# marcelm/cutadapt

Measured on NVIDIA H100. Metric: reads/sec (150bp SE, 1 adapter, e=0.1), higher is better.
Workload: dtype u8

## Files before the change

cutadapt_b200/csrc/cg_core.cuh:

```cuda
#pragma once
#include "cg_types.h"

#define CGK_KIND_ALIGNER 0
#define CGK_KIND_PREFIX 1
#define CGK_KIND_SUFFIX 2
#define CGK_REMOVE_BEFORE 0
#define CGK_REMOVE_AFTER 1
#define CGK_REMOVE_AUTO 2
#define CGK_GROUP_SINGLE 0
#define CGK_GROUP_LINKED 1
#define CGK_GROUP_INDEXED 2

CG_HD int cg_ctz(uint32_t x)
{
#if defined(__CUDA_ARCH__)
    return __ffs((int)x) - 1;
#else
    return __builtin_ctz(x);
#endif
}
CG_HD uint32_t cg_funnel_r(uint32_t lo, uint32_t hi, uint32_t shift_bits)
{
#if defined(__CUDA_ARCH__)
    return __funnelshift_r(lo, hi, shift_bits);
// ... 1697 lines not shown
    locate_regs<MR>(A, ncnt, maxcost, peq, rv, R, R.n, has_task, !split, st);
    if (!has_task) return true;
    if (split && !st.stopped) return false;
    hit_from_state(A, n, st, hit);
    return true;
}

template <int MR>
CG_HD void split_end_pass(const SetView &S, const uint8_t *tail, int n, bool has_task, LocState &st, CgHit &hit)
{
    const CgAdapter &A = S.ad[0];
    const int lo_end = cg_max(0, n - 1 - A.m - A.k);
    ReadView rv;
    rv.n = n; rv.rev = A.reverse;
    rv.p = A.reverse ? tail : tail - lo_end;
    const int32_t *ncnt = (const int32_t *)(S.pool + A.ncount_off);
    const int32_t *maxcost = (const int32_t *)(S.pool + A.maxcost_off);
    const uint32_t *peq = (const uint32_t *)(S.pool + A.peq_off);
    RunList R;
    R.n = 1; R.lo0 = lo_end; R.hi0 = n; R.lo1 = R.hi1 = R.lo2 = R.hi2 = 0;
    locate_regs<MR>(A, ncnt, maxcost, peq, rv, R, 1, has_task, true, st, false);
    if (has_task) hit_from_state(A, n, st, hit);
}

CG_HD void process_read_simple(const SetView &S, const uint8_t *seq, const uint8_t *qual, int n,
                               int quality_trim, int cutoff_front, int cutoff_back, int qbase,
                               PackedCol &colp, cg_match_rec *out, int32_t *qtrim_out, int use_regs = 0)
{
    int s = 0, e = n;
    if (quality_trim) pre_trim_core(seq, qual, n, quality_trim, cutoff_front, cutoff_back, qbase, &s, &e);
    if (qtrim_out) { qtrim_out[0] = s; qtrim_out[1] = e; }
    CgHit hit; hit.adapter = -1; hit.remove = 0;
    hit.astart = hit.astop = hit.rstart = hit.rstop = hit.score = hit.errors = 0;
    if (use_regs == 3 && S.ad[0].m <= 32) {
        int gs3;
        const ScanOut sc3 = simple_scan(S, seq + s, e - s, &gs3);
        if (sc3.pass) {
            LocState st;
            const CgAdapter &A = S.ad[0];
            const int nn = e - s, lo_end = cg_max(0, nn - 1 - A.m - A.k);
            const uint8_t *tail = A.reverse ? seq + s : seq + s + lo_end;
            if (A.m <= 16) {
                if (!split_main_pass<16>(S, seq + s, nn, sc3.hits, gs3, sc3.rs0, sc3.rs1, true, hit, st))
                    split_end_pass<16>(S, tail, nn, true, st, hit);
            } else {
                if (!split_main_pass<32>(S, seq + s, nn, sc3.hits, gs3, sc3.rs0, sc3.rs1, true, hit, st))
                    split_end_pass<32>(S, tail, nn, true, st, hit);
            }
        }
        store_hit(out, hit, 0, e - s);
        return;
    }
    if (use_regs == 2 && S.ad[0].m <= 32) {
        RunList R;
        if (simple_scan_runs(S, seq + s, e - s, R)) {
            if (!simple_locate_runs(S, seq + s, e - s, R, true, hit)) hit.adapter = -1;
        }
        store_hit(out, hit, 0, e - s);
        return;
    }
    int gs;
    const ScanOut sc = simple_scan(S, seq + s, e - s, &gs);
    if (sc.pass) {
        const bool found = (use_regs && S.ad[0].m <= 32)
                               ? simple_locate_regs(S, seq + s, e - s, sc.hits, gs, sc.rs0, sc.rs1, true, hit)
                               : simple_locate(S, seq + s, e - s, sc.hits, gs, colp, hit);
        if (!found) hit.adapter = -1;
    }
    store_hit(out, hit, 0, e - s);
}




struct RunPlan {
    int n_runs;
    int lo0, hi0, lo1, hi1, lo2, hi2, lo3, hi3;
    int end_idx;
    int exact;
    int s0;
    int banded;
};

CG_HD int run_band_d(const CgAdapter &A, int n, int lo, int hi, bool hit_derived, bool is_end_run)
{
    const bool can = A.m <= 64 && !(A.flags & 1) && (A.flags & 2) && (A.flags & 8) && A.indel_cost == 1;
    if (!can || !hit_derived || is_end_run || hi >= n) return -1;
    const int d = hi - A.m - A.k - lo;
    return d >= 0 ? d : -1;
}

template <bool REV>
CG_HD void plan_hit_runs_dir(const CgScanWord *words, int n_words, const uint8_t *pool, const CgAdapter &A,
                             const uint8_t *first, int n, uint32_t hits, int gs, uint32_t rs0, uint32_t rs1,
                             bool want_exact, RunList &R, int &exact, int &s0_out)
{
    const int m = A.m, k = A.k;
    R.n = 0;
    R.lo0 = R.hi0 = R.lo1 = R.hi1 = R.lo2 = R.hi2 = 0;
    exact = 0; s0_out = 0;
    if (A.flags & 1) runs_add(R, 0, cg_min(n, m + k), n);
    if (!hits) return;
    int n_loc = 0;
    for (int w = 0; w < n_words; ++w) n_loc += (words[w].type == CG_SCAN_WHOLE && words[w].loc_found) ? 1 : 0;
    bool ex_ok = want_exact;
    int ex_s0 = -1;
    for (int w = 0; w < n_words; ++w) {
        const CgScanWord &W = words[w];
        if (W.type != CG_SCAN_WHOLE || !W.loc_found) continue;
        CG_TABPTR(mask, (const uint32_t *)(pool + W.mask_off));
        CG_CHARPTR(ltab, pool + W.loc_off);
        const uint32_t init = W.init, locf = W.loc_found;
        const bool stash = n_loc == 1;
        uint32_t todo = hits, Rr = 0;
        int cur_p = -1, nh = 0, stretch = 0;
        int wlo = 0x3fffffff, whi = -1;
        int s0 = 0x3fffffff;
        uint32_t fm = 0;
        while (todo) {
            const int g = cg_ctz(todo);
            todo &= todo - 1;
            const int p_first = g << gs;
            const long long p_end_ll = ((long long)(g + 1)) << gs;
            const int p_end = p_end_ll > n ? n : (int)p_end_ll;
            if (cur_p != p_first) {
                if (cur_p >= 0) ++stretch;
                if (whi >= 0) { runs_add(R, wlo, whi, n); wlo = 0x3fffffff; whi = -1; }
                if (stash && nh < 2) {
                    Rr = nh == 0 ? rs0 : rs1;
                } else {
                    Rr = 0;
                    const int q0 = cg_max(0, p_first - 31);
                    CG_CHARPTR(q, first + (REV ? -q0 : q0));
                    for (int i = q0; i < p_first; ++i) {
                        Rr = ((Rr << 1) | init) & CG_TAB32(mask, CG_CHAR(q));
                        q = REV ? q - 1 : q + 1;
                    }
                }
            }
            ++nh;
            uint32_t q0 = 0, q1 = 0, q2 = 0, q3 = 0, qpa = 0, qpb = 0;
            int qn = 0;
            auto handle = [&](int p, uint32_t f) {
                while (f) {
                    const int b = cg_ctz(f);
                    f &= f - 1;
                    const int bmin = (int)CG_CHAR(ltab + 2 * b), bmax = (int)CG_CHAR(ltab + 2 * b + 1);
                    wlo = cg_min(wlo, p + 1 - bmax - k);
                    whi = cg_max(whi, p + 1 - bmin + m + k);
                    if (stretch == 0) {
                        const int s = p + 1 - bmin;
                        if (s < s0) { s0 = s; fm = 1u << b; }
                        else if (s == s0) fm |= 1u << b;
                    }
                }
            };
            auto flush = [&]() {
                for (int e = qn - 1; e >= 0; --e) {
                    const uint32_t f = e == 3 ? q3 : (e == 2 ? q2 : (e == 1 ? q1 : q0));
                    const uint32_t pw = e >= 2 ? qpb : qpa;
                    handle((int)((e & 1) ? (pw >> 16) : (pw & 0xffffu)), f);
                }
                qn = 0;
            };
            auto push = [&](int p, uint32_t f) {
                if (qn == 4) flush();
                q3 = q2; q2 = q1; q1 = q0; q0 = f;
                qpb = (qpb << 16) | (qpa >> 16);
                qpa = (qpa << 16) | (uint32_t)p;
                ++qn;
            };
            CG_CHARPTR(q, first + (REV ? -p_first : p_first));
            for (int p = p_first; p < p_end; ++p) {
                Rr = ((Rr << 1) | init) & CG_TAB32(mask, CG_CHAR(q));
                q = REV ? q - 1 : q + 1;
                const uint32_t f = Rr & locf;
                if (f) push(p, f);
            }
            flush();
            cur_p = p_end;
        }
        if (whi >= 0) runs_add(R, wlo, whi, n);
        if (fm == locf && s0 >= 0 && s0 + m <= n && (ex_s0 < 0 || ex_s0 == s0)) ex_s0 = s0;
        else ex_ok = false;
    }
    if (ex_ok && ex_s0 >= 0) { exact = 1; s0_out = ex_s0; }
}

template <class T>
CG_HD void plan_runs_myers_t(const CgAdapter &A, const uint32_t *peq, const int32_t *ncnt,
                             const int32_t *maxcost, const uint8_t *p, int n, RunList &R, bool &need_end)
{
    const int m = A.m, k = A.k;
    const bool sir = (A.flags & 1) != 0, eir = (A.flags & 4) != 0;
    const T mmask = m >= (int)(8 * sizeof(T)) ? (T) ~(T)0 : (T)(((T)1 << m) - 1);
    const T top = (T)1 << (m - 1);
    T Pv = sir ? (T)0 : mmask, Mv = 0;
    int score = sir ? 0 : m;
    CG_CHARPTR(cp, A.reverse ? p + (n - 1) : p);
    CG_TABPTR(peq_t, peq);
    const int cstride = A.reverse ? -1 : 1;
    int wlo = 0, whi = -1;
    for (int j = 1; j <= n; ++j) {
        const int ch = (int)(CG_CHAR(cp + cstride * (j - 1)) & 127u);
        T Eq = (T)CG_TAB32(peq_t, ch);
        if (sizeof(T) > 4) Eq |= (T)((unsigned long long)CG_TAB32(peq_t, 128 + ch) << 32);
        const T Xv = Eq | Mv;
        const T Xh = (T)((((Eq & Pv) + Pv) ^ Pv) | Eq);
        T Ph = (T)(Mv | ~(Xh | Pv));
        T Mh = Pv & Xh;
        score += (Ph & top) ? 1 : 0;
        score -= (Mh & top) ? 1 : 0;
        Ph = (T)(Ph << 1); Mh = (T)(Mh << 1);
        Pv = (T)(Mh | ~(Xv | Ph));
        Mv = Ph & Xv;
        if (score <= k) {
            const int lo = cg_max(0, j - m - k);
            if (whi < 0) wlo = lo;
            else if (lo > whi) { runs_add(R, wlo, whi, n); wlo = lo; }
            whi = j;
        }
    }
    if (whi >= 0) runs_add(R, wlo, whi, n);
    need_end = false;
    if (eir) {
        if (sir) need_end = true;
        else {
            int c = 0;
            for (int i = 1; i <= m; ++i) {
                c += (int)((Pv >> (i - 1)) & 1) - (int)((Mv >> (i - 1)) & 1);
                int eff = i;
                if (A.wildcard_ref) eff = (i < m) ? i - ncnt[i] : A.effective_length;
                if (i >= A.min_overlap && c <= maxcost[eff]) { need_end = true; break; }
            }
        }
    }
}

template <class T>
CG_HD int end_overlap_myers_t(const CgAdapter &A, const uint32_t *peq, const int32_t *ncnt,
                              const int32_t *maxcost, const uint8_t *p, int n, int lo_end)
{
    const int m = A.m;
    const T mmask = m >= (int)(8 * sizeof(T)) ? (T) ~(T)0 : (T)(((T)1 << m) - 1);
    T Pv = mmask, Mv = 0;
    CG_CHARPTR(cp, A.reverse ? p + (n - 1) : p);
    CG_TABPTR(peq_t, peq);
    const int cstride = A.reverse ? -1 : 1;
    for (int j = lo_end + 1; j <= n; ++j) {
        const int ch = (int)(CG_CHAR(cp + cstride * (j - 1)) & 127u);
        T Eq = (T)CG_TAB32(peq_t, ch);
        if (sizeof(T) > 4) Eq |= (T)((unsigned long long)CG_TAB32(peq_t, 128 + ch) << 32);
        const T Xv = Eq | Mv;
        const T Xh = (T)((((Eq & Pv) + Pv) ^ Pv) | Eq);
        T Ph = (T)(Mv | ~(Xh | Pv));
        T Mh = Pv & Xh;
        Ph = (T)(Ph << 1); Mh = (T)(Mh << 1);
        Pv = (T)(Mh | ~(Xv | Ph));
        Mv = Ph & Xv;
    }
    int c = 0, best = 0;
    bool inexact = false;
    for (int i = 1; i <= m; ++i) {
        c += (int)((Pv >> (i - 1)) & 1) - (int)((Mv >> (i - 1)) & 1);
        int eff = i;
        if (A.wildcard_ref) eff = (i < m) ? i - ncnt[i] : A.effective_length;
        if (i >= A.min_overlap && c <= maxcost[eff]) {
            if (c == 0) best = i; else inexact = true;
        }
    }
    return inexact ? -1 : best;
}

template <class T>
CG_HD bool run_has_candidate_t(const CgAdapter &A, const uint32_t *peq, const uint8_t *p, int n, int lo, int hi)
{
    const int m = A.m, k = A.k;
    const T mmask = m >= (int)(8 * sizeof(T)) ? (T) ~(T)0 : (T)(((T)1 << m) - 1);
    const T top = (T)1 << (m - 1);
    T Pv = mmask, Mv = 0;
    int score = m;
    CG_CHARPTR(cp, A.reverse ? p + (n - 1) : p);
    CG_TABPTR(peq_t, peq);
    const int cstride = A.reverse ? -1 : 1;
    bool any = false;
    for (int j = lo + 1; j <= hi; ++j) {
        const int ch = (int)(CG_CHAR(cp + cstride * (j - 1)) & 127u);
        T Eq = (T)CG_TAB32(peq_t, ch);
        if (sizeof(T) > 4) Eq |= (T)((unsigned long long)CG_TAB32(peq_t, 128 + ch) << 32);
        const T Xv = Eq | Mv;
        const T Xh = (T)((((Eq & Pv) + Pv) ^ Pv) | Eq);
        T Ph = (T)(Mv | ~(Xh | Pv));
        T Mh = Pv & Xh;
        score += (Ph & top) ? 1 : 0;
        score -= (Mh & top) ? 1 : 0;
        Ph = (T)(Ph << 1); Mh = (T)(Mh << 1);
        Pv = (T)(Mh | ~(Xv | Ph));
        Mv = Ph & Xv;
        any = any || score <= k;
    }
    return any;
}

CG_HD void plan_finish(const SetView &S, const uint8_t *p, int n, const RunList &R0, RunPlan &P, bool skip_end = false)
{
    const CgAdapter &A = S.ad[0];
    const int32_t *ncnt = (const int32_t *)(S.pool + A.ncount_off);
    const int32_t *maxcost = (const int32_t *)(S.pool + A.maxcost_off);
    const uint32_t *peq = (const uint32_t *)(S.pool + A.peq_off);
    const bool eir = (A.flags & 4) != 0;
    const int lo_end = cg_max(0, n - 1 - A.m - A.k);
    const bool can_filter = A.m <= 64 && !(A.flags & 1) && (A.flags & 2) && (A.flags & 8) && A.indel_cost == 1;
    RunList R;
    R.n = 0; R.lo0 = R.hi0 = R.lo1 = R.hi1 = R.lo2 = R.hi2 = 0;
    bool covered = false;
    for (int r = 0; r < R0.n; ++r) {
        const int lo = r == 0 ? R0.lo0 : (r == 1 ? R0.lo1 : R0.lo2);
        const int hi = r == 0 ? R0.hi0 : (r == 1 ? R0.hi1 : R0.hi2);
        const bool is_final = eir && r == R0.n - 1 && lo <= lo_end && hi == n;
        bool keep = true;
        if (can_filter && !is_final)
            keep = A.m <= 32 ? run_has_candidate_t<uint32_t>(A, peq, p, n, lo, hi)
                             : run_has_candidate_t<unsigned long long>(A, peq, p, n, lo, hi);
        if (!keep) continue;
        if (R.n == 0) { R.lo0 = lo; R.hi0 = hi; }
        else if (R.n == 1) { R.lo1 = lo; R.hi1 = hi; }
        else { R.lo2 = lo; R.hi2 = hi; }
        ++R.n;
        covered = is_final;
    }
    P.n_runs = R.n; P.lo0 = R.lo0; P.hi0 = R.hi0; P.lo1 = R.lo1; P.hi1 = R.hi1; P.lo2 = R.lo2; P.hi2 = R.hi2;
    if (!eir || covered || skip_end) return;
    if (can_filter) {
        const int r = A.m <= 32 ? end_overlap_myers_t<uint32_t>(A, peq, ncnt, maxcost, p, n, lo_end)
                                : end_overlap_myers_t<unsigned long long>(A, peq, ncnt, maxcost, p, n, lo_end);
        if (r == 0) return;
        if (r > 0 && R.n == 0) { P.exact = 2; P.s0 = r; return; }
    }
    P.end_idx = R.n;
    if (R.n == 0) { P.lo0 = lo_end; P.hi0 = n; }
    else if (R.n == 1) { P.lo1 = lo_end; P.hi1 = n; }
    else if (R.n == 2) { P.lo2 = lo_end; P.hi2 = n; }
    else { P.lo3 = lo_end; P.hi3 = n; }
    P.n_runs = R.n + 1;
}

CG_HD void plan_runs(const SetView &S, const uint8_t *p, int n, uint32_t hits, int gs, uint32_t rs0,
                     uint32_t rs1, RunPlan &P)
{
    const CgAdapter &A = S.ad[0];
    P.n_runs = 0; P.lo0 = P.hi0 = P.lo1 = P.hi1 = P.lo2 = P.hi2 = P.lo3 = P.hi3 = 0;
    P.end_idx = -1; P.exact = 0; P.s0 = 0; P.banded = 0;
    if (S.h->myers && (A.flags & 2) && (A.flags & 8) && n > 0) {
        const int32_t *ncnt = (const int32_t *)(S.pool + A.ncount_off);
        const int32_t *maxcost = (const int32_t *)(S.pool + A.maxcost_off);
        const uint32_t *peq = (const uint32_t *)(S.pool + A.peq_off);
        RunList R;
        R.n = 0; R.lo0 = R.hi0 = R.lo1 = R.hi1 = R.lo2 = R.hi2 = 0;
        bool need_end;
        if (A.m <= 32) plan_runs_myers_t<uint32_t>(A, peq, ncnt, maxcost, p, n, R, need_end);
        else plan_runs_myers_t<unsigned long long>(A, peq, ncnt, maxcost, p, n, R, need_end);
        P.n_runs = R.n; P.lo0 = R.lo0; P.hi0 = R.hi0; P.lo1 = R.lo1; P.hi1 = R.hi1; P.lo2 = R.lo2; P.hi2 = R.hi2;
        if (need_end) {
            const int lo_end = cg_max(0, n - 1 - A.m - A.k);
            bool covered = false;
            if (R.n > 0) {
                const int lo_last = R.n == 1 ? R.lo0 : (R.n == 2 ? R.lo1 : R.lo2);
                const int hi_last = R.n == 1 ? R.hi0 : (R.n == 2 ? R.hi1 : R.hi2);
                covered = lo_last <= lo_end && hi_last == n;
            }
            if (!covered) {
                P.end_idx = R.n;
                if (R.n == 0) { P.lo0 = lo_end; P.hi0 = n; }
                else if (R.n == 1) { P.lo1 = lo_end; P.hi1 = n; }
                else if (R.n == 2) { P.lo2 = lo_end; P.hi2 = n; }
                else { P.lo3 = lo_end; P.hi3 = n; }
                P.n_runs = R.n + 1;
            }
        }
        return;
    }
    if (!simple_windowed(S, n)) {
        int max_n = n, min_n = 0;
        if (!(A.flags & 2)) max_n = cg_min(n, A.m + A.k);
        if (!(A.flags & 8)) min_n = cg_max(0, n - A.m - A.k);
        P.n_runs = 1; P.lo0 = min_n; P.hi0 = max_n;
        return;
    }
    RunList R;
    const bool want_exact = S.h->exact_ok != 0;
    if (A.reverse) plan_hit_runs_dir<true>(S.scan, S.h->scan_count, S.pool, A, p + (n - 1), n, hits, gs, rs0, rs1, want_exact, R, P.exact, P.s0);
    else plan_hit_runs_dir<false>(S.scan, S.h->scan_count, S.pool, A, p, n, hits, gs, rs0, rs1, want_exact, R, P.exact, P.s0);
    if (P.exact) return;
    plan_finish(S, p, n, R, P);
}

CG_HD bool window_is_plain(const uint8_t *p, int n)
{
    if (n <= 0) return true;
    const uint32_t mis = (uint32_t)((uintptr_t)p & 3u);
    const int total = n + (int)mis;
    const int n_words = (total + 3) >> 2;
#if defined(__CUDA_ARCH__)
    const uint32_t base = (uint32_t)__cvta_generic_to_shared(p - mis);
#define CG_PLAIN_WORD(i) cg_lds_u32(base + 4u * (uint32_t)(i))
#else
    const uint8_t *base = p - mis;
#define CG_PLAIN_WORD(i) ((uint32_t)base[4 * (i)] | ((uint32_t)base[4 * (i) + 1] << 8) | ((uint32_t)base[4 * (i) + 2] << 16) | \
                          ((uint32_t)base[4 * (i) + 3] << 24))
#endif
    uint32_t hi_or = 0, lo_or = 0, six_and = 0xFFFFFFFFu;
    auto take = [&](uint32_t w) {
        const uint32_t s1 = w >> 1, s2 = w >> 2, s4 = w >> 4;
        hi_or |= w & 0x88888888u;
        six_and &= w;
        lo_or |= ((s2 & ~s1) ^ s4) | ~(w ^ s4);
    };
    uint32_t keep0 = 0xFFFFFFFFu << (8 * mis);
    const uint32_t keep_last = (total & 3) ? 0xFFFFFFFFu >> (8 * (4 - (total & 3))) : 0xFFFFFFFFu;
    if (n_words == 1) keep0 &= keep_last;
    take((CG_PLAIN_WORD(0) & keep0) | (0x41414141u & ~keep0));
#pragma unroll 4
    for (int i = 1; i < n_words - 1; ++i) take(CG_PLAIN_WORD(i));
    if (n_words > 1) take((CG_PLAIN_WORD(n_words - 1) & keep_last) | (0x41414141u & ~keep_last));
#undef CG_PLAIN_WORD
    return hi_or == 0 && (six_and & 0x40404040u) == 0x40404040u && (lo_or & 0x01010101u) == 0;
}

CG_HD void plan_runs_planes(const SetView &S, const uint8_t *p, int n, const uint32_t *M, int W, int end_hit,
                            int no_end, int off0, RunPlan &P)
{
    const CgAdapter &A = S.ad[0];
    P.n_runs = 0; P.lo0 = P.hi0 = P.lo1 = P.hi1 = P.lo2 = P.hi2 = P.lo3 = P.hi3 = 0;
    P.end_idx = -1; P.exact = 0; P.s0 = 0; P.banded = 1;
    RunList R;
    R.n = 0; R.lo0 = R.hi0 = R.lo1 = R.hi1 = R.lo2 = R.hi2 = 0;
    if (A.flags & 1) runs_add(R, 0, cg_min(n, A.m + A.k), n);
#pragma unroll
    for (int b = 0; b < 8; ++b) {
        uint32_t x = b < W ? M[b] : 0u;
        while (x) {
            const int e = 32 * b + cg_ctz(x);
            x &= x - 1;
            const int s = e - (A.m - 1) - off0;
            runs_add(R, s - A.k, s + A.m + A.k, n);
        }
    }
    if (end_hit) runs_add(R, cg_max(0, n - 1 - A.m - A.k), n, n);
    plan_finish(S, p, n, R, P, no_end != 0 && !end_hit);
}

CG_HD void hit_end_overlap(const CgAdapter &A, int n, int len, CgHit &hit)
{
    LocState st = loc_state_init(A.m, n);
    st.have = 1; st.b_origin = n - len; st.b_cost = 0; st.b_score = len; st.b_ref_stop = len; st.b_q_stop = n;
    hit_from_state(A, n, st, hit);
}

CG_HD void hit_exact(const CgAdapter &A, int n, int s0, CgHit &hit)
{
    hit.adapter = 0;
    if (A.reverse) { hit.astart = 0; hit.astop = A.m; hit.rstart = n - (s0 + A.m); hit.rstop = n - s0; }
    else { hit.astart = 0; hit.astop = A.m; hit.rstart = s0; hit.rstop = s0 + A.m; }
    hit.score = A.m; hit.errors = 0;
    hit.remove = A.remove == CGK_REMOVE_AUTO ? (hit.rstart == 0 ? CGK_REMOVE_BEFORE : CGK_REMOVE_AFTER)
                                            : A.remove;
}

template <int MR>
CG_HD void run_pass(const SetView &S, const uint8_t *bytes, int n, int lo, int hi, bool eval_bottom,
                    bool final_scan, bool has_task, LocState &st, int band_d = -1)
{
    const CgAdapter &A = S.ad[0];
    ReadView rv;
    rv.n = n; rv.rev = A.reverse;
    rv.p = A.reverse ? bytes - (n - hi) : bytes - lo;
    const int32_t *ncnt = (const int32_t *)(S.pool + A.ncount_off);
    const int32_t *maxcost = (const int32_t *)(S.pool + A.maxcost_off);
    const uint32_t *peq = (const uint32_t *)(S.pool + A.peq_off);
    RunList R;
    R.n = 1; R.lo0 = lo; R.hi0 = hi; R.lo1 = R.hi1 = R.lo2 = R.hi2 = 0;
    if (MR <= 16 && (A.flags & 2)) locate_regs<MR, true, true, CG_RUN_BAND != 0>(A, ncnt, maxcost, peq, rv, R, 1, has_task, final_scan, st, eval_bottom, band_d);
    else locate_regs<MR, false, true, CG_RUN_BAND != 0>(A, ncnt, maxcost, peq, rv, R, 1, has_task, final_scan, st, eval_bottom, band_d);
}

CG_HD void finish_planned(const SetView &S, const uint8_t *w, int nn, const RunPlan &P, CgHit &hit)
{
    const CgAdapter &A = S.ad[0];
    if (P.exact == 2) hit_end_overlap(A, nn, P.s0, hit);
    else if (P.exact) hit_exact(A, nn, P.s0, hit);
    else {
        LocState st = loc_state_init(A.m, nn);
        for (int r = 0; r < P.n_runs && !st.stopped; ++r) {
            const int lo = r == 0 ? P.lo0 : (r == 1 ? P.lo1 : (r == 2 ? P.lo2 : P.lo3));
            const int hi = r == 0 ? P.hi0 : (r == 1 ? P.hi1 : (r == 2 ? P.hi2 : P.hi3));
            const uint8_t *bytes = A.reverse ? w + (nn - hi) : w + lo;
            const bool last = r == P.n_runs - 1;
            const int band = run_band_d(A, nn, lo, hi, P.banded != 0, r == P.end_idx);
            if (A.m <= 16) run_pass<16>(S, bytes, nn, lo, hi, r != P.end_idx, last, true, st, band);
            else if (A.m <= 32) run_pass<32>(S, bytes, nn, lo, hi, r != P.end_idx, last, true, st, band);
            else if (A.m <= 48) run_pass<48>(S, bytes, nn, lo, hi, r != P.end_idx, last, true, st, band);
            else run_pass<64>(S, bytes, nn, lo, hi, r != P.end_idx, last, true, st, band);
        }
        hit_from_state(A, nn, st, hit);
    }
}

CG_HD void process_read_planned(const SetView &S, const uint8_t *seq, const uint8_t *qual, int n,
                                int quality_trim, int cutoff_front, int cutoff_back, int qbase,
                                cg_match_rec *out, int32_t *qtrim_out)
{
    int s = 0, e = n;
    if (quality_trim) pre_trim_core(seq, qual, n, quality_trim, cutoff_front, cutoff_back, qbase, &s, &e);
    if (qtrim_out) { qtrim_out[0] = s; qtrim_out[1] = e; }
    CgHit hit; hit.adapter = -1; hit.remove = 0;
    hit.astart = hit.astop = hit.rstart = hit.rstop = hit.score = hit.errors = 0;
    const CgAdapter &A = S.ad[0];
    const int nn = e - s;
    int gs;
    const ScanOut sc = simple_scan(S, seq + s, nn, &gs);
    if (sc.pass) {
        RunPlan P;
        plan_runs(S, seq + s, nn, sc.hits, gs, sc.rs0, sc.rs1, P);
        finish_planned(S, seq + s, nn, P, hit);
    }
    store_hit(out, hit, 0, nn);
}

CG_HD const uint32_t *plane_program(const SetView &S)
{
    return (const uint32_t *)((const uint8_t *)S.h + S.h->plane_off);
}

CG_HD void process_read_planes(const SetView &S, const uint8_t *seq, const uint8_t *qual, int n,
                               int quality_trim, int cutoff_front, int cutoff_back, int qbase,
                               cg_match_rec *out, int32_t *qtrim_out)
{
    int s = 0, e = n;
    if (quality_trim) pre_trim_core(seq, qual, n, quality_trim, cutoff_front, cutoff_back, qbase, &s, &e);
    if (qtrim_out) { qtrim_out[0] = s; qtrim_out[1] = e; }
    const CgAdapter &A = S.ad[0];
    const int nn = e - s;
    if (S.h->plane_count > 0 && nn >= 1 && nn <= 256) {
        const uint8_t *ref = S.pool + A.ref_off;
        const PlaneOut po = nn <= 160
            ? plane_scan_core<5, RuntimePlaneProg>(plane_program(S), S.h->plane_count, S.h->plane_flags, A.m, ref, seq + e, nn, A.pf_count == 0)
            : plane_scan_core<8, RuntimePlaneProg>(plane_program(S), S.h->plane_count, S.h->plane_flags, A.m, ref, seq + e, nn, A.pf_count == 0);
        if (po.cls != CG_PLANE_SLOW) {
            CgHit hit; hit.adapter = -1; hit.remove = 0;
            hit.astart = hit.astop = hit.rstart = hit.rstop = hit.score = hit.errors = 0;
            if (po.cls == CG_PLANE_EXACT) hit_exact(A, nn, po.s0, hit);
            else if (po.cls == CG_PLANE_OVERLAP) hit_end_overlap(A, nn, po.s0, hit);
            store_hit(out, hit, 0, nn);
            return;
        }
        if (window_is_plain(seq + s, nn)) {
            const int W = nn <= 160 ? 5 : 8;
            RunPlan P;
            plan_runs_planes(S, seq + s, nn, po.M, W, po.end_hit, po.no_end, 32 * W - nn, P);
            CgHit hit; hit.adapter = -1; hit.remove = 0;
            hit.astart = hit.astop = hit.rstart = hit.rstop = hit.score = hit.errors = 0;
            finish_planned(S, seq + s, nn, P, hit);
            store_hit(out, hit, 0, nn);
            return;
        }
    }
    process_read_planned(S, seq + s, nullptr, nn, 0, 0, 0, qbase, out, nullptr);
}
```

Before: 7.391 billion.

## Use Wu-Manber bit-parallel filter for short adapters with small error budgets

Adds Wu-Manber (Shift-And with k error rows) variants of the candidate filter and end-overlap check, specialized at compile time for k=0,1,2 when the adapter fits in 32 bits. They replace Myers' bit-vector score tracking for these cases and are meant to reduce per-column arithmetic and branching in the prefilter. The cost is more code paths, with a risk of semantic mismatch against the Myers version (initial states R1=1, R2=3, max-cost row selection).

```diff
diff --git a/cutadapt_b200/csrc/cg_core.cuh b/cutadapt_b200/csrc/cg_core.cuh
--- a/cutadapt_b200/csrc/cg_core.cuh
+++ b/cutadapt_b200/csrc/cg_core.cuh
@@ -2023,6 +2023,57 @@
     return any;
 }
 
+template <int K>
+CG_HD void wm_column(uint32_t &R0, uint32_t &R1, uint32_t &R2, uint32_t Eq)
+{
+    const uint32_t o0 = R0, o1 = R1;
+    R0 = ((o0 << 1) | 1u) & Eq;
+    if (K >= 1) R1 = (((o1 << 1) | 1u) & Eq) | o0 | ((o0 | R0) << 1) | 1u;
+    if (K >= 2) R2 = (((R2 << 1) | 1u) & Eq) | o1 | ((o1 | R1) << 1) | 1u;
+}
+
+template <int K>
+CG_HD bool run_has_candidate_wm(const CgAdapter &A, const uint32_t *peq, const uint8_t *p, int n, int lo, int hi)
+{
+    uint32_t R0 = 0, R1 = 1u, R2 = 3u, acc = 0;
+    CG_CHARPTR(cp, A.reverse ? p + (n - 1) : p);
+    CG_TABPTR(peq_t, peq);
+    const int cstride = A.reverse ? -1 : 1;
+    for (int j = lo + 1; j <= hi; ++j) {
+        const int ch = (int)(CG_CHAR(cp + cstride * (j - 1)) & 127u);
+        wm_column<K>(R0, R1, R2, CG_TAB32(peq_t, ch));
+        acc |= K == 0 ? R0 : (K == 1 ? R1 : R2);
+    }
+    return ((acc >> (A.m - 1)) & 1u) != 0;
+}
+
+template <int K>
+CG_HD int end_overlap_wm(const CgAdapter &A, const uint32_t *peq, const int32_t *ncnt, const int32_t *maxcost,
+                         const uint8_t *p, int n, int lo_end)
+{
+    const int m = A.m;
+    uint32_t R0 = 0, R1 = 1u, R2 = 3u;
+    CG_CHARPTR(cp, A.reverse ? p + (n - 1) : p);
+    CG_TABPTR(peq_t, peq);
+    const int cstride = A.reverse ? -1 : 1;
+    for (int j = lo_end + 1; j <= n; ++j) {
+        const int ch = (int)(CG_CHAR(cp + cstride * (j - 1)) & 127u);
+        wm_column<K>(R0, R1, R2, CG_TAB32(peq_t, ch));
+    }
+    int best = 0;
+    bool inexact = false;
+    for (int i = A.min_overlap > 1 ? A.min_overlap : 1; i <= m; ++i) {
+        const int eff = A.wildcard_ref ? ((i < m) ? i - ncnt[i] : A.effective_length) : i;
+        const int mc = maxcost[eff];
+        if (mc < 0) continue;
+        const uint32_t Rm = mc == 0 ? R0 : (mc == 1 || K == 1 ? R1 : R2);
+        if ((Rm >> (i - 1)) & 1u) {
+            if ((R0 >> (i - 1)) & 1u) best = i; else inexact = true;
+        }
+    }
+    return inexact ? -1 : best;
+}
+
 CG_HD void plan_finish(const SetView &S, const uint8_t *p, int n, const RunList &R0, RunPlan &P, bool skip_end = false)
 {
     const CgAdapter &A = S.ad[0];
@@ -2032,6 +2083,7 @@
     const bool eir = (A.flags & 4) != 0;
     const int lo_end = cg_max(0, n - 1 - A.m - A.k);
     const bool can_filter = A.m <= 64 && !(A.flags & 1) && (A.flags & 2) && (A.flags & 8) && A.indel_cost == 1;
+    const int wm_k = (A.m <= 32 && A.k >= 0 && A.k <= 2 && A.k < A.m) ? A.k : -1;
     RunList R;
     R.n = 0; R.lo0 = R.hi0 = R.lo1 = R.hi1 = R.lo2 = R.hi2 = 0;
     bool covered = false;
@@ -2041,7 +2093,10 @@
         const bool is_final = eir && r == R0.n - 1 && lo <= lo_end && hi == n;
         bool keep = true;
         if (can_filter && !is_final)
-            keep = A.m <= 32 ? run_has_candidate_t<uint32_t>(A, peq, p, n, lo, hi)
+            keep = wm_k == 0 ? run_has_candidate_wm<0>(A, peq, p, n, lo, hi)
+                 : wm_k == 1 ? run_has_candidate_wm<1>(A, peq, p, n, lo, hi)
+                 : wm_k == 2 ? run_has_candidate_wm<2>(A, peq, p, n, lo, hi)
+                 : A.m <= 32 ? run_has_candidate_t<uint32_t>(A, peq, p, n, lo, hi)
                              : run_has_candidate_t<unsigned long long>(A, peq, p, n, lo, hi);
         if (!keep) continue;
         if (R.n == 0) { R.lo0 = lo; R.hi0 = hi; }
@@ -2053,7 +2108,10 @@
     P.n_runs = R.n; P.lo0 = R.lo0; P.hi0 = R.hi0; P.lo1 = R.lo1; P.hi1 = R.hi1; P.lo2 = R.lo2; P.hi2 = R.hi2;
     if (!eir || covered || skip_end) return;
     if (can_filter) {
-        const int r = A.m <= 32 ? end_overlap_myers_t<uint32_t>(A, peq, ncnt, maxcost, p, n, lo_end)
+        const int r = wm_k == 0 ? end_overlap_wm<0>(A, peq, ncnt, maxcost, p, n, lo_end)
+                    : wm_k == 1 ? end_overlap_wm<1>(A, peq, ncnt, maxcost, p, n, lo_end)
+                    : wm_k == 2 ? end_overlap_wm<2>(A, peq, ncnt, maxcost, p, n, lo_end)
+                    : A.m <= 32 ? end_overlap_myers_t<uint32_t>(A, peq, ncnt, maxcost, p, n, lo_end)
                                 : end_overlap_myers_t<unsigned long long>(A, peq, ncnt, maxcost, p, n, lo_end);
         if (r == 0) return;
         if (r > 0 && R.n == 0) { P.exact = 2; P.s0 = r; return; }
```

Result: faster. 7.493 billion, median of 6 (+1.4%).
